# lgemc/WildlifeMapper

Measured on AMD Instinct MI355X. Metric: 1024x1024 tiles/sec (whole node), higher is better.
Workload: dtype fp16; 1 GPU; vit_h full path fft+encoder+decoder+PostProcess/NMS, fp16 MFMA, batch=16 tiles/GPU of 1024x1024x3 (BASELINE.json configs[2]); parallelism=dp1 tile shard, weights=seed 0 synthetic (random init), tolerance=logits within 1e-3 relative of the fp32 CPU forward, identical NMS index lists

## Files before the change

include/wm_hip.h:

```cpp
#ifndef WM_HIP_H
#define WM_HIP_H

#include <stdint.h>

#ifdef __cplusplus
extern "C" {
#endif

#define WM_ABI_VERSION 13

#define WM_PREC_BF16 0
#define WM_PREC_FP16 1
#define WM_PREC_FP8 2

#define WM_MAX_GLOBAL 8
#define WM_NUM_QUERIES 51
#define WM_NUM_LOGITS 8

typedef struct wm_config {
    int32_t embed_dim;
    int32_t depth;
    int32_t num_heads;
    int32_t num_global;
    int32_t global_attn_indexes[WM_MAX_GLOBAL];
// ... 32 lines not shown
int wm_abi_version(void);

int wm_create(const wm_config* cfg, int device, wm_handle** out);
int wm_destroy(wm_handle* h);
int wm_load_weight(wm_handle* h, const char* name, const float* host_data,
                   const int64_t* shape, int ndim);
int wm_finalize_weights(wm_handle* h);


int wm_preprocess_u8(const uint8_t* img_dev, float* out_dev, int batch, int height, int width, void* stream);

int wm_preprocess_u8_resized(const uint8_t* img_dev, float* out_dev, int batch, int height, int width, int size, int max_size,
                             void* stream);
int wm_resized_size(int height, int width, int size, int max_size, int* out_h, int* out_w);
int wm_debug_resize_coeffs(int in_size, int out_size, int* bounds_out, int* kk_out, int kk_capacity, int* ksize_out);

int wm_hfc_fft(wm_handle* h, const float* x_dev, float* hfc_dev, int batch, void* stream);

int wm_encoder_forward(wm_handle* h, const float* x_dev, const float* hfc_dev,
                       float* out_dev, int batch, void* stream);

int wm_decoder_forward(wm_handle* h, const float* emb_dev, float* logits_dev,
                       float* boxes_dev, int batch, void* stream);

int wm_postprocess_nms(wm_handle* h, const float* logits_dev, const float* boxes_dev,
                       const float* target_sizes_dev, float conf_thr, float score_thr,
                       float iou_thr, wm_box_record* records_dev, int batch, void* stream);

int wm_forward(wm_handle* h, const float* x_dev, const float* target_sizes_dev,
               float* logits_dev, float* boxes_dev, wm_box_record* records_dev,
               int batch, void* stream);

#define WM_CRITERION_MAX_TARGETS 2048
#define WM_CRITERION_SUMS 8
#define WM_CRITERION_NONFINITE 1
#define WM_CRITERION_UNSOLVED 2
int64_t wm_criterion_scratch_bytes(int batch, int total_targets);
int wm_criterion(wm_handle* h, const float* logits_dev, const float* boxes_dev, const float* tgt_boxes_dev,
                 const int32_t* tgt_labels_dev, const int32_t* tgt_offsets, int batch, float w_class, float w_bbox, float w_giou,
                 float eos_coef, void* scratch_dev, int64_t scratch_bytes, int32_t* match_dev, double* sums_dev,
                 int32_t* status_dev, float* cost_dev, double* dual_u_dev, double* dual_v_dev, void* stream);

typedef struct wm_frame_desc {
    const uint8_t* data;
    int32_t height, width;
} wm_frame_desc;
// ... 182 lines not shown
```

wildlifemapper_amd/_native.py:

```python
from __future__ import annotations

import ctypes as C
import os
from typing import Optional

import torch

_HERE = os.path.dirname(os.path.abspath(__file__))
LIB_PATH = os.environ.get("WM_HIP_LIB") or os.path.join(_HERE, "libwm_hip.so")

PREC_BF16, PREC_FP16, PREC_FP8 = 0, 1, 2
PREC_BY_NAME = {"bf16": PREC_BF16, "fp16": PREC_FP16, "f16": PREC_FP16, "fp8": PREC_FP8}
NUM_QUERIES, NUM_LOGITS = 51, 8
KCLASS_NAMES = ("gemm16", "attn_window", "attn_global", "layernorm", "other")
GEMM_VARIANTS = ("v1_128", "v2_160", "v2_128", "v3_lockstep", "v3_conv3x3", "v5_320", "v5_320_res", "v5_256", "v5_256_res",
                 "v5_320_lnf", "v5_256_lnf", "fp8_320", "fp8_256", "v5_320_foldp", "v5_256_foldp", "v5_320_split", "v5_256_split", "v3_patch_embed", "fp8_256_planes")
FLAG_CONF, FLAG_SCORE, FLAG_NMS, FLAG_MERGED = 1, 2, 4, 8
CRITERION_MAX_TARGETS, CRITERION_SUMS, CRITERION_NONFINITE, CRITERION_UNSOLVED = 2048, 8, 1, 2
CENSUS_MAX_DETS, CENSUS_SAME_CLASS, CENSUS_UNSOLVED = 262144, 1, 1
COVERAGE_MAX_SIDE, COVERAGE_MAX_CELLS, COVERAGE_MAX_FRAMES, COVERAGE_CLASSES, COVERAGE_STATS = 16384, 1 << 26, 65535, 7, 16
CFG_FUSE_LN = 1
CFG_FOLD_LN = 2
CFG_FOLD_LN_BF16 = 4
ABI_VERSION = 13
# ... 29 lines not shown
    "wm_finalize_weights": (_I, [_P]),
    "wm_preprocess_u8": (_I, [_P, _P, _I, _I, _I, _P]),
    "wm_preprocess_u8_resized": (_I, [_P, _P, _I, _I, _I, _I, _I, _P]),
    "wm_resized_size": (_I, [_I, _I, _I, _I, C.POINTER(_I), C.POINTER(_I)]),
    "wm_debug_resize_coeffs": (_I, [_I, _I, C.POINTER(_I), C.POINTER(_I), _I, C.POINTER(_I)]),
    "wm_tile_frames_u8": (_I, [_P, _I, _P, _P, _I, _P]),
    "wm_merge_frames_scratch_bytes": (_L, [_I]),
    "wm_merge_frames_nms": (_I, [_P, _P, C.POINTER(C.c_int32), _I, _F, _P, _L, _P, _P, _P, _P, _P]),
    "wm_merge_frames_fuse": (_I, [_P, _P, C.POINTER(C.c_int32), _I, _F, _P, _L, _P, _P, _P, _P, _P, _P, _P]),
    "wm_census_scratch_bytes": (_L, [_I]),
    "wm_census": (_I, [_P, _P, _P, _P, _I, _P, _I, C.c_double, _I, _P, _L, _P, _P, _P, _P, _P, _P]),
    "wm_coverage_raster": (_I, [_P, _P, _I, C.c_double, C.c_double, C.c_double, _I, _I, _P, _P, _P]),
    "wm_coverage_points": (_I, [_P, _P, _I, _P, _P, _I, C.c_double, C.c_double, C.c_double, _I, _I, _P, _P, _P, _P, _P]),
    "wm_resample_u8": (_I, [_P, _I, _I, _P, _I, _I, _P]),
    "wm_scaled_size": (_I, [_I, _I, C.c_double, C.POINTER(_I), C.POINTER(_I)]),
    "wm_chip_window": (_I, [C.POINTER(_F), _F, _I, _I, C.POINTER(C.c_int32)]),
    "wm_crop_chips_u8": (_I, [_P, _I, _P, _P, _I, _I, _F, _I, _I, _P, _P, _P]),
    "wm_box_outline_rect": (_I, [C.POINTER(_F), C.POINTER(C.c_int32)]),
    "wm_draw_boxes_u8": (_I, [_P, _I, _P, _P, _P, _I, _P, _I, _I, _P]),
    "wm_plot_image_u8": (_I, [_P, _I, _I, _I, _P, _P, _L, _P]),
    "wm_hfc_fft": (_I, [_P, _P, _P, _I, _P]),
    "wm_encoder_forward": (_I, [_P, _P, _P, _P, _I, _P]),
    "wm_decoder_forward": (_I, [_P, _P, _P, _P, _I, _P]),
    "wm_postprocess_nms": (_I, [_P, _P, _P, _P, _F, _F, _F, _P, _I, _P]),
    "wm_criterion_scratch_bytes": (_L, [_I, _I]),
    "wm_criterion": (_I, [_P, _P, _P, _P, _P, C.POINTER(C.c_int32), _I, _F, _F, _F, _F, _P, _L, _P, _P, _P, _P, _P, _P, _P]),
    "wm_forward": (_I, [_P, _P, _P, _P, _P, _P, _I, _P]),
    "wm_set_tap": (_I, [_P, _I]),
    "wm_read_tap": (_I, [_P, _P, _I, _P]),
    "wm_profile_enable": (_I, [_P, _I]),
    "wm_profile_reset": (_I, [_P]),
    "wm_profile_read": (_I, [_P, C.POINTER(WmKclassStat)]),
    "wm_debug_gemm_variant_counts": (_I, [C.POINTER(_L), _I]),
    "wm_debug_reset_gemm_variant_counts": (_I, []),
    "wm_debug_saturation_enable": (_I, [_P, _I]),
    "wm_debug_saturation_read": (_I, [_P, C.POINTER(_L), _I, _I, _P]),
    "wm_op_cvt_f32_to_16": (_I, [_P, _P, _L, _I, _P]),
    "wm_op_cvt_16_to_f32": (_I, [_P, _P, _L, _I, _P]),
    "wm_op_gemm16": (_I, [_P, _P, _P, _P, _I, _P, _P, _I, _I, _I, _I, _I, _P]),
    "wm_op_gemm16_takes_packed": (_I, [_I, _I, _I]),
    "wm_op_pack16": (_I, [_P, _P, _L, _I, _P]),
    "wm_op_ln_stats16": (_I, [_P, _P, _P, _L, _I, _I, _P]),
    "wm_op_ln_stats16_split": (_I, [_P, _P, _P, _P, _P, _L, _I, _I, _P]),
    "wm_op_gemm16_split": (_I, [_P, _P, _P, _P, _P, _P, _I, _I, _I, _I, _I, _P]),
    "wm_op_stream_merge": (_I, [_P, _P, _P, _L, _I, _I, _P]),
    "wm_op_unpack16": (_I, [_P, _P, _L, _I, _P]),
# ... 71 lines not shown
```

wildlifemapper_amd/csrc/gemm32.h:

```cpp
#pragma once
#include "wm_common.h"
#include "gemm_common.h"

namespace wm {

struct Gemm32Args {
    const float* A; const float* W; const float* bias; const float* residual; float* out;
    int M, N, K, act;
    int lda;
};

__global__ __launch_bounds__(256) void gemm32_kernel(Gemm32Args p) {
    constexpr int BM = 64, BN = 64, BK = 32, LD = BK + 1;
    __shared__ float sA[BM * LD];
    __shared__ float sW[BN * LD];
    const int tid = threadIdx.x, lane = tid & 63, wave = tid >> 6;
    const int wr = wave >> 1, wc = wave & 1;
    const int ntn = (p.N + BN - 1) / BN;
    const int lid = xcd_remap(blockIdx.x, gridDim.x);
    const int m0 = (lid / ntn) * BM, n0 = (lid % ntn) * BN;
    const int lrow = tid >> 2, lcol = (tid & 3) * 8;

    f32x16 acc;
#pragma unroll
// ... 30 lines not shown
    if (n >= p.N) return;
    const float bv = p.bias ? p.bias[n] : 0.f;
#pragma unroll
    for (int r = 0; r < 16; ++r) {
        const int m = m0 + wr * 32 + (r & 3) + 8 * (r >> 2) + 4 * (lane >> 5);
        if (m < p.M) {
            float v = acc[r] + bv;
            if (p.act == ACT_RELU) v = fmaxf(v, 0.f);
            else if (p.act == ACT_GELU) v = gelu_erf(v);
            else if (p.act == ACT_SIGMOID) v = 1.0f / (1.0f + expf(-v));
            if (p.residual) v += p.residual[(size_t)m * p.N + n];
            p.out[(size_t)m * p.N + n] = v;
        }
    }
}

constexpr float G32X3_WSCALE = 64.0f;
constexpr float G32X3_LOSCALE = 2048.0f;
struct Gemm32x3Args {
    const float* A; const float* W; const u16* Whi; const u16* Wlo;
    const float* bias; const float* residual; float* out;
    int M, N, K, act, lda;
    int* overflow;
};

__global__ __launch_bounds__(256) void split_w32_kernel(const float* __restrict__ w, u16* __restrict__ hi, u16* __restrict__ lo, int64_t n4, int* overflow) {
    for (int64_t i = (int64_t)blockIdx.x * 256 + threadIdx.x; i < n4; i += (int64_t)gridDim.x * 256) {
        const f32x4 v = *(const f32x4*)(w + i * 4) * G32X3_WSCALE;
        typename FP16::vec4 h, l;
        float amax = 0.f;
#pragma unroll
        for (int j = 0; j < 4; ++j) {
            h[j] = FP16::from_f32_bounded(v[j]);
            l[j] = FP16::from_f32_bounded((v[j] - FP16::to_f32(h[j])) * G32X3_LOSCALE);
            amax = fmaxf(amax, fabsf(v[j]));
        }
        *(typename FP16::vec4*)(hi + i * 4) = h;
        *(typename FP16::vec4*)(lo + i * 4) = l;
        if (amax >= 65504.f && overflow) *(volatile int*)overflow = 1;
    }
}

template <bool WPRE>
__global__ __launch_bounds__(256) void gemm32x3_kernel(Gemm32x3Args p) {
    constexpr int BM = 64, BN = 64, BK = 32, LDH = BK + 8;
    __shared__ __attribute__((aligned(16))) u16 sAh[BM * LDH], sAl[BM * LDH], sWh[BN * LDH], sWl[BN * LDH];
// ... 45 lines not shown
        else split8(s.w0, s.w1, G32X3_WSCALE, wh, wl);
        __syncthreads();
        *(uint4*)(sAh + lrow * LDH + lcol) = ah; *(uint4*)(sAl + lrow * LDH + lcol) = al;
        *(uint4*)(sWh + lrow * LDH + lcol) = wh; *(uint4*)(sWl + lrow * LDH + lcol) = wl;
        __syncthreads();
        if (kt + 2 < nk) fetch(s, (kt + 2) * BK);
#pragma unroll
        for (int ks = 0; ks < 2; ++ks) {
            const typename FP16::vec8 a_hi = *(const typename FP16::vec8*)(sAh + fa + 16 * ks), a_lo = *(const typename FP16::vec8*)(sAl + fa + 16 * ks);
            const typename FP16::vec8 w_hi = *(const typename FP16::vec8*)(sWh + fw + 16 * ks), w_lo = *(const typename FP16::vec8*)(sWl + fw + 16 * ks);
            accx = FP16::mfma32(a_lo, w_hi, accx);
            accx = FP16::mfma32(a_hi, w_lo, accx);
            acc = FP16::mfma32(a_hi, w_hi, acc);
        }
    };
    for (int kt = 0; kt < nk; kt += 2) {
        step(st[0], kt);
        if (kt + 1 < nk) step(st[1], kt + 1);
    }
    if (amax >= 65504.f && p.overflow) *(volatile int*)p.overflow = 1;

    const int n = n0 + wc * 32 + (lane & 31);
    if (n >= p.N) return;
    const float bv = p.bias ? p.bias[n] : 0.f;
#pragma unroll
    for (int r = 0; r < 16; ++r) {
        const int m = m0 + wr * 32 + (r & 3) + 8 * (r >> 2) + 4 * (lane >> 5);
        if (m < p.M) {
            float v = (acc[r] + accx[r] * (1.0f / G32X3_LOSCALE)) * (1.0f / G32X3_WSCALE) + bv;
            if (p.act == ACT_RELU) v = fmaxf(v, 0.f);
            else if (p.act == ACT_GELU) v = gelu_erf(v);
            else if (p.act == ACT_SIGMOID) v = 1.0f / (1.0f + expf(-v));
            if (p.residual) v += p.residual[(size_t)m * p.N + n];
            p.out[(size_t)m * p.N + n] = v;
        }
    }
}

}
```

wildlifemapper_amd/csrc/host_core.h:

```cpp
#pragma once
#include <hip/hip_runtime.h>

#include <cmath>
#include <cstdarg>
#include <cstdio>
#include <cstdlib>
#include <cstring>
#include <atomic>
#include <map>
#include <tuple>
#include <type_traits>
#include <mutex>
#include <set>
#include <string>
#include <algorithm>
#include <array>
#include <vector>

#include "../../include/wm_hip.h"
#include "wm_common.h"

#ifndef WM_DEV_TIMELINE
#define WM_DEV_TIMELINE 0
#endif
// ... 168 lines not shown
    std::map<const float*, std::pair<uint16_t*, uint16_t*>> w32x3;
    std::map<std::pair<const float*, int>, uint16_t*> bias16;
    float* mha_part = nullptr;
    size_t mha_part_cap = 0;
    bool row_major = false;
    bool sat_on = false;
    unsigned long long* sat_counts = nullptr;
    int tap_which = -2;
    float* tap_buf = nullptr;

    float *resid = nullptr, *tokbase = nullptr;
    uint16_t *xn16 = nullptr, *ao16 = nullptr, *qkv16 = nullptr, *hid16 = nullptr;
    uint16_t *p16 = nullptr, *h16 = nullptr, *he16 = nullptr, *hp16 = nullptr, *pt16 = nullptr, *q16 = nullptr,
             *kv16 = nullptr, *aoh16 = nullptr, *y1n16 = nullptr, *h1_16 = nullptr, *y2_16 = nullptr, *y2t16 = nullptr;
    float *pt32 = nullptr, *y1 = nullptr, *y1n32 = nullptr, *z32 = nullptr;
    float *n1 = nullptr, *n2 = nullptr, *emb_nhwc = nullptr, *emb_nchw = nullptr;
    uint16_t *n1n16 = nullptr, *x16last = nullptr;
    float *dkeys = nullptr, *dk_a = nullptr, *dk_b = nullptr, *dk_c = nullptr;
    float *dq = nullptr, *dt_q = nullptr, *dt_k = nullptr, *dt_v = nullptr, *dt_att = nullptr, *dt_hid = nullptr,
          *dt_h1 = nullptr, *dt_h2 = nullptr;
    float *logits = nullptr, *boxes = nullptr, *hfc = nullptr, *tsz_default = nullptr;
    float2 *fftR = nullptr, *fft_tw = nullptr;
    float* kpe = nullptr;
    wm_box_record* records = nullptr;
};

namespace {

template <class P>
int dalloc(wm_handle* h, P** out, size_t bytes) {
    void* p = nullptr;
    hipError_t e = hipMalloc(&p, bytes);
    if (e != hipSuccess) return fail("hipMalloc(%zu) failed: %s", bytes, hipGetErrorString(e));
    h->allocs.push_back(p);
    *out = (P*)p;
    return 0;
}

void dfree(wm_handle* h, void* p) {
    hipFree(p);
    for (auto& a : h->allocs) if (a == p) a = nullptr;
}

struct Bracket {
    wm_handle* h;
    hipStream_t s;
// ... 59 lines not shown
```

wildlifemapper_amd/csrc/host_decoder.h:

```cpp
#pragma once
#include "dec_kernels.h"
#include "host_encoder.h"

namespace {

struct DecAttnW { const float *wq, *bq, *wk, *bk, *wv, *bv, *wo, *bo; int internal; };

DecAttnW dec_w(wm_handle* h, const std::string& p, int internal) {
    return DecAttnW{W32(h, p + "q_proj.weight"), W32(h, p + "q_proj.bias"), W32(h, p + "k_proj.weight"), W32(h, p + "k_proj.bias"),
                    W32(h, p + "v_proj.weight"), W32(h, p + "v_proj.bias"), W32(h, p + "out_proj.weight"), W32(h, p + "out_proj.bias"), internal};
}

int decoder_impl(wm_handle* h, const float* keys_nhwc, float* logits, float* boxes, int B, hipStream_t s) {
    const std::string t = "mask_decoder.transformer.";
    const int E = OUTC, Mk = B * T, Mq = B * NQ;
    const float* tok = W32(h, "mask_decoder.mask_tokens.weight");
    float* keys = h->dkeys;
    HIP_TRY(hipMemcpyAsync(keys, keys_nhwc, (size_t)Mk * E * 4, hipMemcpyDeviceToDevice, s));
    float* queries = h->dq;
    WM_TRY(launch_simple(h, s, 0.0, add_bcast_kernel, dim3(grid_for((int64_t)Mq * E / 4)), dim3(256), (const float*)nullptr, tok, queries, (int64_t)Mq, E, NQ));

    auto add_q = [&](float* out) {
        return launch_simple(h, s, 0.0, add_bcast_kernel, dim3(grid_for((int64_t)Mq * E / 4)), dim3(256), (const float*)queries, tok, out, (int64_t)Mq, E, NQ);
    };
    auto add_k = [&](float* out) {
        return launch_simple(h, s, 0.0, add_bcast_kernel, dim3(grid_for((int64_t)Mk * E / 4)), dim3(256), (const float*)keys, (const float*)h->kpe, out, (int64_t)Mk, E, T);
    };
    auto ln = [&](float* x, const std::string& n, int rows) {
        return launch_layernorm(h, s, WM_PREC_FP16, x, W32(h, n + ".weight"), W32(h, n + ".bias"), 1e-5f, x, nullptr, rows, E);
    };
    auto token_to_image = [&](const DecAttnW& w, const float* kin) -> int {
        WM_TRY(add_q(h->dt_h1));
        WM_TRY(launch_gemm32(h, s, h->dt_h1, w.wq, w.bq, nullptr, h->dt_q, Mq, w.internal, E, ACT_NONE));
        WM_TRY(launch_gemm32(h, s, kin, w.wk, w.bk, nullptr, h->dk_a, Mk, w.internal, E, ACT_NONE));
        WM_TRY(launch_gemm32(h, s, keys, w.wv, w.bv, nullptr, h->dk_b, Mk, w.internal, E, ACT_NONE));
        WM_TRY(launch_mha32(h, s, h->dt_q, h->dk_a, h->dk_b, h->dt_att, B, 8, w.internal / 8, NQ, T));
// ... 26 lines not shown
            WM_TRY(add_q(h->dt_h1));
            WM_TRY(launch_gemm32(h, s, kpe_sum, w.wq, w.bq, nullptr, h->dk_a, Mk, w.internal, E, ACT_NONE));
            WM_TRY(launch_gemm32(h, s, h->dt_h1, w.wk, w.bk, nullptr, h->dt_k, Mq, w.internal, E, ACT_NONE));
            WM_TRY(launch_gemm32(h, s, queries, w.wv, w.bv, nullptr, h->dt_v, Mq, w.internal, E, ACT_NONE));
            WM_TRY(launch_mha32(h, s, h->dk_a, h->dt_k, h->dt_v, h->dk_c, B, 8, w.internal / 8, T, NQ));
            WM_TRY(launch_gemm32(h, s, h->dk_c, w.wo, w.bo, keys, keys, Mk, E, w.internal, ACT_NONE));
            WM_TRY(ln(keys, L + "norm4", Mk));
        }
    }
    WM_TRY(add_k(kpe_sum));
    WM_TRY(token_to_image(dec_w(h, t + "final_attn_token_to_image.", E / 2), kpe_sum));
    WM_TRY(ln(queries, t + "norm_final_attn", Mq));

    const std::string c = "mask_decoder.class_embed.layers.", bb = "mask_decoder.bbox_embed.layers.";
    WM_TRY(launch_gemm32(h, s, queries, W32(h, c + "0.weight"), W32(h, c + "0.bias"), nullptr, h->dt_h1, Mq, E, E, ACT_RELU));
    WM_TRY(launch_gemm32(h, s, h->dt_h1, W32(h, c + "1.weight"), W32(h, c + "1.bias"), nullptr, h->dt_h2, Mq, E, E, ACT_RELU));
    WM_TRY(launch_gemm32(h, s, h->dt_h2, W32(h, c + "2.weight"), W32(h, c + "2.bias"), nullptr, logits, Mq, WM_NUM_LOGITS, E, ACT_NONE));
    WM_TRY(launch_gemm32(h, s, queries, W32(h, bb + "0.weight"), W32(h, bb + "0.bias"), nullptr, h->dt_h1, Mq, E, E, ACT_RELU));
    WM_TRY(launch_gemm32(h, s, h->dt_h1, W32(h, bb + "1.weight"), W32(h, bb + "1.bias"), nullptr, h->dt_h2, Mq, E, E, ACT_RELU));
    WM_TRY(launch_gemm32(h, s, h->dt_h2, W32(h, bb + "2.weight"), W32(h, bb + "2.bias"), nullptr, boxes, Mq, 4, E, ACT_SIGMOID));
    return 0;
}

int forward_impl(wm_handle* h, const float* x_dev, const float* target_sizes_dev, float* logits_dev, float* boxes_dev,
                 wm_box_record* records_dev, int batch, hipStream_t s) {
    WM_TRY(fft_impl(h, x_dev, h->hfc, batch, s, true));
    WM_TRY(encoder_impl(h, x_dev, h->hfc, nullptr, batch, s, true));
    WM_TRY(decoder_impl(h, h->emb_nhwc, h->logits, h->boxes, batch, s));
    const float* ts = target_sizes_dev ? target_sizes_dev : h->tsz_default;
    WM_TRY(launch_simple(h, s, 0.0, postprocess_nms_kernel, dim3(batch), dim3(64), (const float*)h->logits, (const float*)h->boxes, ts,
                         0.05f, 0.5f, 0.4f, h->records));
    if (logits_dev) HIP_TRY(hipMemcpyAsync(logits_dev, h->logits, (size_t)batch * NQ * WM_NUM_LOGITS * 4, hipMemcpyDeviceToDevice, s));
    if (boxes_dev) HIP_TRY(hipMemcpyAsync(boxes_dev, h->boxes, (size_t)batch * NQ * 16, hipMemcpyDeviceToDevice, s));
    if (records_dev) HIP_TRY(hipMemcpyAsync(records_dev, h->records, (size_t)batch * NQ * sizeof(wm_box_record), hipMemcpyDeviceToDevice, s));
    return 0;
}

}
```

wildlifemapper_amd/csrc/host_gemm.h:

```cpp
#pragma once
#include "gemm16.h"
#include "gemm16_v2.h"
#include "gemm16_v3.h"
#include "gemm16_v5.h"
#include "gemm32.h"
#include "gemm8.h"
#include "misc_kernels.h"
#include "host_core.h"

namespace {

double gemm16_flops(const Gemm16Args& a) { return 2.0 * a.M * (double)a.N * a.K; }
double gemm16_bytes(const Gemm16Args& a) {
    return 2.0 * ((double)a.M * a.K + (double)a.N * a.K) + (a.out32 ? 4.0 : 0.0) * a.M * a.N + (a.out16 ? 2.0 : 0.0) * a.M * a.N +
           (a.residual ? 4.0 * (double)(a.res_mod > 0 ? a.res_mod : a.M) * a.N : 0.0);
}

template <class Kern, class Args>
int launch_gemm_kernel(wm_handle* h, hipStream_t s, Kern kern, int grid, int threads, int lds, const Args& a, int variant, double flops, double bytes) {
    WM_TRY(set_max_lds((const void*)kern, lds));
    if (variant >= 0) count_variant(variant);
    Bracket br(h, s, WM_KCLASS_GEMM16, flops, bytes);
    hipLaunchKernelGGL(kern, dim3(grid), dim3(threads), lds, s, a);
    HIP_TRY(hipGetLastError());
// ... 160 lines not shown
    });
}

int launch_patch_embed16(wm_handle* h, hipStream_t s, int prec, const void* img16, const void* W, const float* bias, const float* res, int res_mod,
                         float* out32, void* out16, int B, int N, int Cin) {
    const int M = B * 4096, K = Cin * 256;
    if (B <= 0 || (N % 320 && N % 256) || Cin <= 0) return fail("patch_embed: B=%d N=%d Cin=%d unsupported (N %% 320 or N %% 256)", B, N, Cin);
    if (!out32 && !out16) return fail("patch_embed: no output");
    Gemm16Args a{};
    a.A = (const u16*)img16; a.W = (const u16*)W; a.bias = bias; a.residual = res; a.out32 = out32; a.out16 = (u16*)out16;
    a.M = M; a.N = N; a.K = K; a.res_mod = res_mod; a.act = ACT_NONE; a.conv_c = Cin;
    count_variant(WM_GEMM_V3_PATCH);
    const double bytes = 2.0 * ((double)M * K + (double)N * K) + (out32 ? 4.0 : 0.0) * M * N + (out16 ? 2.0 : 0.0) * M * N;
    return by_type16(prec, [&](auto t) {
        return by_tile_width(N, [&](auto bn) {
            constexpr int BN = decltype(bn)::value;
            using G = G3<BN>;
            return launch_gemm_kernel(h, s, gemm16v3_kernel<decltype(t), BN, ALoad::PatchEmbed>, (M / 256) * (N / BN), G::THREADS, G::LDS, a, -1,
                                      2.0 * M * (double)N * K, bytes);
        });
    });
}

int launch_gemm32(wm_handle* h, hipStream_t s, const float* A, const float* W, const float* bias, const float* res,
                  float* out, int M, int N, int K, int act, int lda = 0, int mode = 0) {
    if (K % 16) return fail("gemm32: K=%d must be a multiple of 16", K);
    static const bool f32_only = getenv("WM_GEMM32_F32") && atoi(getenv("WM_GEMM32_F32")) != 0;
    if ((mode == 2 || mode == 3) && K % 32) return fail("gemm32 (split form): K=%d must be a multiple of 32", K);
    if (mode == 2 || mode == 3 || (mode == 0 && h && !f32_only && K % 32 == 0)) {
        Gemm32x3Args a{A, W, nullptr, nullptr, bias, res, out, M, N, K, act, lda > 0 ? lda : K, h ? h->overflow + 1 : nullptr};
        if (mode == 3) {
            const size_t n = (size_t)N * K;
            void* pb = nullptr;
            WM_TRY(op_scratch(s, 3, n * 4, &pb));
            u16* hi = (u16*)pb;
            hipLaunchKernelGGL(split_w32_kernel, dim3(grid_for((int64_t)n / 4)), dim3(256), 0, s, W, hi, hi + n, (int64_t)n / 4, (int*)nullptr);
            HIP_TRY(hipGetLastError());
            a.Whi = hi; a.Wlo = hi + n;
        }
        if (mode == 0) {
            auto it = h->w32x3.find(W);
            if (it == h->w32x3.end()) {
                uint16_t *hi = nullptr, *lo = nullptr;
                const size_t n = (size_t)N * K;
                if (n % 4) return fail("gemm32: weight of %zu elements", n);
                WM_TRY(dalloc(h, &hi, n * 2)); WM_TRY(dalloc(h, &lo, n * 2));
                hipLaunchKernelGGL(split_w32_kernel, dim3(grid_for((int64_t)n / 4)), dim3(256), 0, s, W, (u16*)hi, (u16*)lo, (int64_t)n / 4, h->overflow + 1);
                HIP_TRY(hipGetLastError());
                it = h->w32x3.emplace(W, std::make_pair(hi, lo)).first;
            }
            a.Whi = (const u16*)it->second.first; a.Wlo = (const u16*)it->second.second;
        }
        Bracket br(h, s, WM_KCLASS_OTHER, 2.0 * M * (double)N * K, 4.0 * ((double)M * K + (double)M * N) + 4.0 * (double)N * K);
// ... 15 lines not shown
```

wildlifemapper_amd/csrc/host_weights.h:

```cpp
#pragma once
#include "misc_kernels.h"
#include "fft_kernels.h"
#include "host_core.h"

namespace {

bool ends_with(const std::string& s, const char* suf) {
    const size_t n = strlen(suf);
    return s.size() >= n && s.compare(s.size() - n, n, suf) == 0;
}

static inline uint16_t f32_to_bf16_host(float f) {
    uint32_t u;
    memcpy(&u, &f, 4);
    if ((u & 0x7fffffffu) > 0x7f800000u) return (uint16_t)((u >> 16) | 0x40);
    u += 0x7fffu + ((u >> 16) & 1u);
    return (uint16_t)(u >> 16);
}

static inline uint16_t f32_to_f16_host(float f) {
    _Float16 h = (_Float16)fminf(fmaxf(f, -65504.f), 65504.f);
    uint16_t r;
    memcpy(&r, &h, 2);
    return r;
}

static inline uint8_t f32_to_e4m3_host(float f) {
    if (f != f) return 0x7f;
// ... 349 lines not shown
                HIP_TRY(hipMemcpy(d32, w.data.data(), n * 4, hipMemcpyHostToDevice));
                h->wsrc32[name] = d32;
            }
        } else {
            WM_TRY(upload32(h, name, w.data.data(), n));
        }
    }
    if (h->staged.count("prompt_encoder.pe_layer.positional_encoding_gaussian_matrix")) {
        const HostW& g = h->staged["prompt_encoder.pe_layer.positional_encoding_gaussian_matrix"];
        const int F = OUTC / 2;
        std::vector<float> pe((size_t)T * OUTC);
        for (int y = 0; y < GRID; ++y)
            for (int x = 0; x < GRID; ++x) {
                const float cx = 2.0f * ((x + 0.5f) / GRID) - 1.0f, cy = 2.0f * ((y + 0.5f) / GRID) - 1.0f;
                for (int f = 0; f < F; ++f) {
                    float arg = cx * g.data[f] + cy * g.data[F + f];
                    arg = arg * 6.283185307179586f;
                    pe[(size_t)(y * GRID + x) * OUTC + f] = (float)sin((double)arg);
                    pe[(size_t)(y * GRID + x) * OUTC + F + f] = (float)cos((double)arg);
                }
            }
        HIP_TRY(hipMemcpy(h->kpe, pe.data(), pe.size() * 4, hipMemcpyHostToDevice));
    }
    if (h->fold && h->enc_ready) {
        for (int i = 0; i < h->depth; ++i) {
            const std::string b = "image_encoder.blocks." + std::to_string(i) + ".";
            const int P = block_prec(h, i) == WM_PREC_FP8 ? WM_PREC_BF16 : block_prec(h, i);
            const std::pair<const char*, const char*> pairs[] = {{"attn.qkv", "norm1"}, {"mlp.lin1", "norm2"}};
            for (const auto& pr : pairs) {
                const std::string wn = b + pr.first + ".weight";
                if (!h->w16.count(wn)) continue;
                const int N = (int)h->expected.at(wn)[0], K = (int)h->expected.at(wn)[1];
                if (!h->wfold.count(wn)) {
                    uint16_t* wf = nullptr; float *c1 = nullptr, *c2 = nullptr;
                    WM_TRY(dalloc(h, &wf, (size_t)N * K * 2)); WM_TRY(dalloc(h, &c1, (size_t)N * 4)); WM_TRY(dalloc(h, &c2, (size_t)N * 4));
                    h->wfold[wn] = wf; h->fold_c1[wn] = c1; h->fold_c2[wn] = c2;
                }
                const float* g = h->w32.at(b + pr.second + ".weight");
                const float* be = h->w32.at(b + pr.second + ".bias");
                const float* bias = h->w32.at(b + pr.first + ".bias");
                WM_TRY(launch_fold_weight(0, P, h->w16.at(wn), h->fold_from16 ? nullptr : h->wsrc32.at(wn), g, be, bias, h->wfold[wn], h->fold_c1[wn], h->fold_c2[wn], N, K));
            }
        }
    }
    HIP_TRY(hipDeviceSynchronize());
    h->staged.clear();
// ... 6 lines not shown
```

wildlifemapper_amd/csrc/wm_api.hip:

```cpp
#include "host_core.h"
#if WM_DEV_TIMELINE
#include "host_dev_timeline.h"
#endif
#include "host_gemm.h"
#include "host_norm.h"
#include "host_attn.h"
#include "host_weights.h"
#include "host_encoder.h"
#include "host_decoder.h"
#include "host_frontend.h"
#include "host_criterion.h"

extern "C" const char* wm_last_error(void) { return g_err; }
extern "C" int wm_abi_version(void) { return WM_ABI_VERSION; }

extern "C" int wm_create(const wm_config* cfg, int device, wm_handle** out) {
    if (!cfg || !out) return fail("wm_create: null argument");
    if (cfg->embed_dim <= 0 || cfg->num_heads <= 0 || cfg->embed_dim % cfg->num_heads) return fail("wm_create: bad dims");
    if (cfg->depth <= 0 || cfg->depth > 64) return fail("wm_create: depth %d out of range", cfg->depth);
    if (cfg->max_batch <= 0) return fail("wm_create: max_batch must be positive");
    if (cfg->embed_dim % 256 || cfg->embed_dim > 1280) return fail("wm_create: embed_dim %d unsupported (multiple of 256, <= 1280)", cfg->embed_dim);
    const int hd = cfg->embed_dim / cfg->num_heads;
    if (hd != 64 && hd != 80) return fail("wm_create: head_dim %d unsupported (64 or 80)", hd);
    if (cfg->precision != WM_PREC_BF16 && cfg->precision != WM_PREC_FP16 && cfg->precision != WM_PREC_FP8) return fail("wm_create: bad precision");
// ... 75 lines not shown

extern "C" int wm_hfc_fft(wm_handle* h, const float* x_dev, float* hfc_dev, int batch, void* stream) {
    if (!h) return fail("wm_hfc_fft: null handle");
    if (batch <= 0 || batch > h->maxB) return fail("wm_hfc_fft: batch %d outside 1..%d", batch, h->maxB);
    if (!x_dev || !hfc_dev) return fail("wm_hfc_fft: null buffer");
    HIP_TRY(hipSetDevice(h->device));
    return fft_impl(h, x_dev, hfc_dev, batch, (hipStream_t)stream);
}

extern "C" int wm_encoder_forward(wm_handle* h, const float* x_dev, const float* hfc_dev, float* out_dev, int batch, void* stream) {
    WM_TRY(check_ready(h, batch, "wm_encoder_forward", true, false));
    if (!x_dev || !hfc_dev || !out_dev) return fail("wm_encoder_forward: null buffer");
    return encoder_impl(h, x_dev, hfc_dev, out_dev, batch, (hipStream_t)stream);
}

extern "C" int wm_decoder_forward(wm_handle* h, const float* emb_dev, float* logits_dev, float* boxes_dev, int batch, void* stream) {
    WM_TRY(check_ready(h, batch, "wm_decoder_forward", false, true));
    if (!emb_dev || !logits_dev || !boxes_dev) return fail("wm_decoder_forward: null buffer");
    hipStream_t s = (hipStream_t)stream;
    WM_TRY(launch_simple(h, s, batch * 8.4e6, transpose32_kernel, dim3(T / 64, OUTC / 64, batch), dim3(256), emb_dev, h->emb_nhwc, OUTC, T));
    return decoder_impl(h, h->emb_nhwc, logits_dev, boxes_dev, batch, s);
}

extern "C" int wm_postprocess_nms(wm_handle* h, const float* logits_dev, const float* boxes_dev, const float* target_sizes_dev,
                                  float conf_thr, float score_thr, float iou_thr, wm_box_record* records_dev, int batch, void* stream) {
    if (batch <= 0) return fail("wm_postprocess_nms: batch %d", batch);
    if (!logits_dev || !boxes_dev || !target_sizes_dev || !records_dev) return fail("wm_postprocess_nms: null buffer");
    if (h) HIP_TRY(hipSetDevice(h->device));
    return launch_simple(h, (hipStream_t)stream, 0.0, postprocess_nms_kernel, dim3(batch), dim3(64), logits_dev, boxes_dev,
                         target_sizes_dev, conf_thr, score_thr, iou_thr, records_dev);
}

extern "C" int wm_forward(wm_handle* h, const float* x_dev, const float* target_sizes_dev, float* logits_dev, float* boxes_dev,
                          wm_box_record* records_dev, int batch, void* stream) {
    WM_TRY(check_ready(h, batch, "wm_forward", true, true));
    if (!x_dev) return fail("wm_forward: null input");
    return forward_impl(h, x_dev, target_sizes_dev, logits_dev, boxes_dev, records_dev, batch, (hipStream_t)stream);
}

extern "C" int64_t wm_criterion_scratch_bytes(int batch, int total_targets) { return criterion_scratch_bytes(batch, total_targets); }

extern "C" int wm_criterion(wm_handle* h, const float* logits_dev, const float* boxes_dev, const float* tgt_boxes_dev,
                            const int32_t* tgt_labels_dev, const int32_t* tgt_offsets, int batch, float w_class, float w_bbox, float w_giou,
                            float eos_coef, void* scratch_dev, int64_t scratch_bytes, int32_t* match_dev, double* sums_dev,
                            int32_t* status_dev, float* cost_dev, double* dual_u_dev, double* dual_v_dev, void* stream) {
    if (h) HIP_TRY(hipSetDevice(h->device));
// ... 355 lines not shown
```

Baseline: 171.3 tiles/s.

## Precompute decoder positional-encoding projections and fuse K/V projections in mask decoder

Precomputes the weight-only parts of the mask decoder at weight-finalize time: positional-encoding and token projections become per-row addend tables, and the first self-attention over the constant mask tokens runs once into a tokens0 constant. The gemm32 epilogue gains a per-row addend table and a split second output, so each token-to-image K and V projection over the image keys runs as one GEMM instead of separate add and projection passes. This removes redundant per-batch work on the constant path and some launches. In exchange it adds stored tables, a more complex epilogue that preloads residuals, and a rounding order that differs slightly from the reference.

After: 172.0 tiles/s (median of 6 runs). Within noise of the previous version (+0.4%).

```diff
diff --git a/include/wm_hip.h b/include/wm_hip.h
--- a/include/wm_hip.h
+++ b/include/wm_hip.h
@@ -78,6 +78,9 @@
 
 int wm_decoder_forward(wm_handle* h, const float* emb_dev, float* logits_dev,
                        float* boxes_dev, int batch, void* stream);
+
+int wm_debug_decoder_kv(wm_handle* h, int which, const float* keys_dev, float* k_out_dev, float* v_out_dev, int fused,
+                        int batch, void* stream);
 
 int wm_postprocess_nms(wm_handle* h, const float* logits_dev, const float* boxes_dev,
                        const float* target_sizes_dev, float conf_thr, float score_thr,
diff --git a/wildlifemapper_amd/_native.py b/wildlifemapper_amd/_native.py
--- a/wildlifemapper_amd/_native.py
+++ b/wildlifemapper_amd/_native.py
@@ -75,6 +75,7 @@
     "wm_hfc_fft": (_I, [_P, _P, _P, _I, _P]),
     "wm_encoder_forward": (_I, [_P, _P, _P, _P, _I, _P]),
     "wm_decoder_forward": (_I, [_P, _P, _P, _P, _I, _P]),
+    "wm_debug_decoder_kv": (_I, [_P, _I, _P, _P, _P, _I, _I, _P]),
     "wm_postprocess_nms": (_I, [_P, _P, _P, _P, _F, _F, _F, _P, _I, _P]),
     "wm_criterion_scratch_bytes": (_L, [_I, _I]),
     "wm_criterion": (_I, [_P, _P, _P, _P, _P, C.POINTER(C.c_int32), _I, _F, _F, _F, _F, _P, _L, _P, _P, _P, _P, _P, _P, _P]),
diff --git a/wildlifemapper_amd/csrc/gemm32.h b/wildlifemapper_amd/csrc/gemm32.h
--- a/wildlifemapper_amd/csrc/gemm32.h
+++ b/wildlifemapper_amd/csrc/gemm32.h
@@ -76,6 +76,8 @@
     const float* bias; const float* residual; float* out;
     int M, N, K, act, lda;
     int* overflow;
+    const float* rowadd; int rowadd_mod, rowadd_n;
+    float* out2; int nsplit;
 };
 
 __global__ __launch_bounds__(256) void split_w32_kernel(const float* __restrict__ w, u16* __restrict__ hi, u16* __restrict__ lo, int64_t n4, int* overflow) {
@@ -167,19 +169,46 @@
 
     const int n = n0 + wc * 32 + (lane & 31);
     if (n >= p.N) return;
-    const float bv = p.bias ? p.bias[n] : 0.f;
+    const int wave_u = __builtin_amdgcn_readfirstlane(wave);
+    const bool tab = p.rowadd && n0 + (wave_u & 1) * 32 < p.rowadd_n;
+    float add[16];
+    if (tab) {
+        const int mb = (m0 + (wave_u >> 1) * 32) % p.rowadd_mod;
+#pragma unroll
+        for (int r = 0; r < 16; ++r) {
+            int row = mb + (r & 3) + 8 * (r >> 2) + 4 * (lane >> 5);
+            if (row >= p.rowadd_mod) row -= p.rowadd_mod;
+            add[r] = p.rowadd[(size_t)row * p.rowadd_n + n];
+        }
+    } else {
+        const float bv = p.bias ? p.bias[n] : 0.f;
+#pragma unroll
+        for (int r = 0; r < 16; ++r) add[r] = bv;
+    }
+    float rs[16];
+#pragma unroll
+    for (int r = 0; r < 16; ++r) {
+        const int m = min(m0 + wr * 32 + (r & 3) + 8 * (r >> 2) + 4 * (lane >> 5), p.M - 1);
+        rs[r] = p.residual ? p.residual[(size_t)m * p.N + n] : 0.f;
+    }
+    float* op = p.out;
+    int ldo = p.N, no = n;
+    if (p.out2) {
+        if (n >= p.nsplit) { op = p.out2; ldo = p.N - p.nsplit; no = n - p.nsplit; }
+        else ldo = p.nsplit;
+    }
 #pragma unroll
     for (int r = 0; r < 16; ++r) {
         const int m = m0 + wr * 32 + (r & 3) + 8 * (r >> 2) + 4 * (lane >> 5);
         if (m < p.M) {
-            float v = (acc[r] + accx[r] * (1.0f / G32X3_LOSCALE)) * (1.0f / G32X3_WSCALE) + bv;
+            float v = (acc[r] + accx[r] * (1.0f / G32X3_LOSCALE)) * (1.0f / G32X3_WSCALE) + add[r];
             if (p.act == ACT_RELU) v = fmaxf(v, 0.f);
             else if (p.act == ACT_GELU) v = gelu_erf(v);
             else if (p.act == ACT_SIGMOID) v = 1.0f / (1.0f + expf(-v));
-            if (p.residual) v += p.residual[(size_t)m * p.N + n];
-            p.out[(size_t)m * p.N + n] = v;
-        }
-    }
-}
-
-}
+            if (p.residual) v += rs[r];
+            op[(size_t)m * ldo + no] = v;
+        }
+    }
+}
+
+}
diff --git a/wildlifemapper_amd/csrc/host_core.h b/wildlifemapper_amd/csrc/host_core.h
--- a/wildlifemapper_amd/csrc/host_core.h
+++ b/wildlifemapper_amd/csrc/host_core.h
@@ -214,6 +214,8 @@
     float *logits = nullptr, *boxes = nullptr, *hfc = nullptr, *tsz_default = nullptr;
     float2 *fftR = nullptr, *fft_tw = nullptr;
     float* kpe = nullptr;
+    std::map<std::string, float*> dconst;
+    std::set<std::string> dconst_bad;
     wm_box_record* records = nullptr;
 };
 
diff --git a/wildlifemapper_amd/csrc/host_dec_tables.h b/wildlifemapper_amd/csrc/host_dec_tables.h
--- /dev/null
+++ b/wildlifemapper_amd/csrc/host_dec_tables.h
@@ -0,0 +1,62 @@
+#pragma once
+#include <string>
+#include <vector>
+
+namespace wm_dec {
+
+enum Kind { KEY_TABLE, TOKEN_TABLE, CONCAT_W, CONCAT_B, TOKENS0 };
+
+struct Derived {
+    Kind kind;
+    std::string key;
+    std::vector<std::string> src;
+    int n;
+};
+
+inline const char* gaussian_name() { return "prompt_encoder.pe_layer.positional_encoding_gaussian_matrix"; }
+inline const char* tokens_name() { return "mask_decoder.mask_tokens.weight"; }
+inline const char* tokens0_key() { return "mask_decoder.tokens0"; }
+inline std::string table_key(const std::string& proj) { return proj + ".pe_const"; }
+inline std::string concat_key(const std::string& attn, const char* what) { return attn + "kv_proj." + what; }
+
+inline std::vector<std::string> token_to_image_attns() {
+    const std::string t = "mask_decoder.transformer.";
+    return {t + "layers.0.cross_attn_token_to_image.", t + "layers.1.cross_attn_token_to_image.", t + "final_attn_token_to_image."};
+}
+
+inline std::vector<Derived> plan(int embed = 256) {
+    const std::string t = "mask_decoder.transformer.";
+    std::vector<Derived> p;
+    auto table = [&](Kind k, const std::string& proj, int n) {
+        p.push_back(Derived{k, table_key(proj), {proj + ".weight", proj + ".bias", k == KEY_TABLE ? gaussian_name() : tokens_name()}, n});
+    };
+    for (const std::string& a : token_to_image_attns()) {
+        table(KEY_TABLE, a + "k_proj", embed / 2);
+        table(TOKEN_TABLE, a + "q_proj", embed / 2);
+        p.push_back(Derived{CONCAT_W, concat_key(a, "weight"), {a + "k_proj.weight", a + "v_proj.weight"}, embed});
+        p.push_back(Derived{CONCAT_B, concat_key(a, "bias"), {a + "k_proj.bias", a + "v_proj.bias"}, embed});
+    }
+    for (int i = 0; i < 2; ++i) {
+        const std::string a = t + "layers." + std::to_string(i) + ".cross_attn_image_to_token.";
+        table(KEY_TABLE, a + "q_proj", embed / 2);
+        table(TOKEN_TABLE, a + "k_proj", embed / 2);
+    }
+    table(TOKEN_TABLE, t + "layers.1.self_attn.q_proj", embed);
+    table(TOKEN_TABLE, t + "layers.1.self_attn.k_proj", embed);
+    Derived t0{TOKENS0, tokens0_key(), {tokens_name()}, embed};
+    for (const char* n : {"q_proj", "k_proj", "v_proj", "out_proj"})
+        for (const char* w : {".weight", ".bias"}) t0.src.push_back(t + "layers.0.self_attn." + n + w);
+    for (const char* w : {".weight", ".bias"}) t0.src.push_back(t + "layers.0.norm1" + w);
+    p.push_back(t0);
+    return p;
+}
+
+template <class Staged, class Built>
+bool stale(const Derived& d, const Staged& staged, const Built& built) {
+    if (!built.count(d.key)) return true;
+    for (const std::string& s : d.src)
+        if (staged.count(s)) return true;
+    return false;
+}
+
+}
diff --git a/wildlifemapper_amd/csrc/host_decoder.h b/wildlifemapper_amd/csrc/host_decoder.h
--- a/wildlifemapper_amd/csrc/host_decoder.h
+++ b/wildlifemapper_amd/csrc/host_decoder.h
@@ -11,7 +11,7 @@
                     W32(h, p + "v_proj.weight"), W32(h, p + "v_proj.bias"), W32(h, p + "out_proj.weight"), W32(h, p + "out_proj.bias"), internal};
 }
 
-int decoder_impl(wm_handle* h, const float* keys_nhwc, float* logits, float* boxes, int B, hipStream_t s) {
+int decoder_unfused_impl(wm_handle* h, const float* keys_nhwc, float* logits, float* boxes, int B, hipStream_t s) {
     const std::string t = "mask_decoder.transformer.";
     const int E = OUTC, Mk = B * T, Mq = B * NQ;
     const float* tok = W32(h, "mask_decoder.mask_tokens.weight");
@@ -84,6 +84,146 @@
     return 0;
 }
 
+const float* DCONST(wm_handle* h, const std::string& n) { return h->dconst.at(n); }
+
+int dec_self_attn0(wm_handle* h, hipStream_t s, float* queries, int B) {
+    const std::string L = "mask_decoder.transformer.layers.0.";
+    const int E = OUTC, Mq = B * NQ;
+    const DecAttnW w = dec_w(h, L + "self_attn.", E);
+    WM_TRY(launch_gemm32(h, s, queries, w.wq, w.bq, nullptr, h->dt_q, Mq, E, E, ACT_NONE));
+    WM_TRY(launch_gemm32(h, s, queries, w.wk, w.bk, nullptr, h->dt_k, Mq, E, E, ACT_NONE));
+    WM_TRY(launch_gemm32(h, s, queries, w.wv, w.bv, nullptr, h->dt_v, Mq, E, E, ACT_NONE));
+    WM_TRY(launch_mha32(h, s, h->dt_q, h->dt_k, h->dt_v, h->dt_att, B, 8, E / 8, NQ, NQ));
+    WM_TRY(launch_gemm32(h, s, h->dt_att, w.wo, w.bo, nullptr, queries, Mq, E, E, ACT_NONE));
+    return launch_layernorm(h, s, WM_PREC_FP16, queries, W32(h, L + "norm1.weight"), W32(h, L + "norm1.bias"), 1e-5f, queries, nullptr, Mq, E);
+}
+
+int dec_build_derived(wm_handle* h) {
+    if (gemm32_f32_only()) return 0;
+    const hipStream_t s = 0;
+    const int E = OUTC;
+    for (const wm_dec::Derived& d : wm_dec::plan(E)) {
+        if (!wm_dec::stale(d, h->staged, h->dconst)) continue;
+        const int rows = d.kind == wm_dec::KEY_TABLE ? T : d.kind == wm_dec::CONCAT_W ? d.n : d.kind == wm_dec::CONCAT_B ? 1 : NQ;
+        const int cols = d.kind == wm_dec::CONCAT_W ? E : d.n;
+        if (!h->dconst.count(d.key)) {
+            float* p = nullptr;
+            WM_TRY(dalloc(h, &p, (size_t)rows * cols * 4));
+            h->dconst[d.key] = p;
+        }
+        float* out = h->dconst.at(d.key);
+        HIP_TRY(hipDeviceSynchronize());
+        volatile int* ovf = (volatile int*)h->overflow + 1;
+        const int ovf_before = *ovf;
+        *ovf = 0;
+        switch (d.kind) {
+            case wm_dec::KEY_TABLE:
+            case wm_dec::TOKEN_TABLE:
+                WM_TRY(launch_gemm32(h, s, d.kind == wm_dec::KEY_TABLE ? h->kpe : W32(h, wm_dec::tokens_name()), W32(h, d.src[0]), W32(h, d.src[1]),
+                                     nullptr, out, rows, d.n, E, ACT_NONE));
+                break;
+            case wm_dec::CONCAT_W:
+            case wm_dec::CONCAT_B: {
+                const size_t half = (size_t)rows * cols / 2 * 4;
+                HIP_TRY(hipMemcpyAsync(out, W32(h, d.src[0]), half, hipMemcpyDeviceToDevice, s));
+                HIP_TRY(hipMemcpyAsync((char*)out + half, W32(h, d.src[1]), half, hipMemcpyDeviceToDevice, s));
+                break;
+            }
+            case wm_dec::TOKENS0:
+                HIP_TRY(hipMemcpyAsync(out, W32(h, wm_dec::tokens_name()), (size_t)NQ * E * 4, hipMemcpyDeviceToDevice, s));
+                WM_TRY(dec_self_attn0(h, s, out, 1));
+                break;
+        }
+        HIP_TRY(hipDeviceSynchronize());
+        if (*ovf) h->dconst_bad.insert(d.key);
+        else h->dconst_bad.erase(d.key);
+        *ovf = ovf_before;
+    }
+    return 0;
+}
+
+int dec_project_kv(wm_handle* h, hipStream_t s, const std::string& attn, const float* keys, float* k_out, float* v_out, int Mk, bool fused) {
+    const int E = OUTC, I = E / 2;
+    Gemm32Ext x;
+    x.rowadd = DCONST(h, wm_dec::table_key(attn + "k_proj")); x.rowadd_mod = T; x.rowadd_n = I;
+    if (!fused) {
+        WM_TRY(launch_gemm32(h, s, keys, W32(h, attn + "k_proj.weight"), nullptr, nullptr, k_out, Mk, I, E, ACT_NONE, 0, 0, &x));
+        return launch_gemm32(h, s, keys, W32(h, attn + "v_proj.weight"), W32(h, attn + "v_proj.bias"), nullptr, v_out, Mk, I, E, ACT_NONE);
+    }
+    x.out2 = v_out; x.nsplit = I;
+    return launch_gemm32(h, s, keys, DCONST(h, wm_dec::concat_key(attn, "weight")), DCONST(h, wm_dec::concat_key(attn, "bias")), nullptr, k_out,
+                         Mk, E, E, ACT_NONE, 0, 0, &x);
+}
+
+int decoder_impl(wm_handle* h, const float* keys_nhwc, float* logits, float* boxes, int B, hipStream_t s) {
+    if (gemm32_f32_only()) return decoder_unfused_impl(h, keys_nhwc, logits, boxes, B, s);
+    const std::string t = "mask_decoder.transformer.";
+    const int E = OUTC, Mk = B * T, Mq = B * NQ;
+    const float* keys = keys_nhwc;
+    float* queries = h->dq;
+    if (!h->dconst_bad.empty()) ((volatile int*)h->overflow)[1] = 1;
+    WM_TRY(launch_simple(h, s, 0.0, add_bcast_kernel, dim3(grid_for((int64_t)Mq * E / 4)), dim3(256), (const float*)nullptr,
+                         DCONST(h, wm_dec::tokens0_key()), queries, (int64_t)Mq, E, NQ));
+
+    auto ln = [&](float* x, const std::string& n, int rows) {
+        return launch_layernorm(h, s, WM_PREC_FP16, x, W32(h, n + ".weight"), W32(h, n + ".bias"), 1e-5f, x, nullptr, rows, E);
+    };
+    auto proj_pe = [&](const float* a, const std::string& proj, int per, float* out, int M, int N) {
+        Gemm32Ext x;
+        x.rowadd = DCONST(h, wm_dec::table_key(proj)); x.rowadd_mod = per; x.rowadd_n = N;
+        return launch_gemm32(h, s, a, W32(h, proj + ".weight"), nullptr, nullptr, out, M, N, E, ACT_NONE, 0, 0, &x);
+    };
+    auto token_to_image = [&](const std::string& a) -> int {
+        const DecAttnW w = dec_w(h, a, E / 2);
+        WM_TRY(proj_pe(queries, a + "q_proj", NQ, h->dt_q, Mq, w.internal));
+        WM_TRY(dec_project_kv(h, s, a, keys, h->dk_a, h->dk_b, Mk, true));
+        WM_TRY(launch_mha32(h, s, h->dt_q, h->dk_a, h->dk_b, h->dt_att, B, 8, w.internal / 8, NQ, T));
+        WM_TRY(launch_gemm32(h, s, h->dt_att, w.wo, w.bo, queries, queries, Mq, E, w.internal, ACT_NONE));
+        return 0;
+    };
+
+    for (int i = 0; i < 2; ++i) {
+        const std::string L = t + "layers." + std::to_string(i) + ".";
+        if (i != 0) {
+            const std::string a = L + "self_attn.";
+            const DecAttnW w = dec_w(h, a, E);
+            WM_TRY(proj_pe(queries, a + "q_proj", NQ, h->dt_q, Mq, E));
+            WM_TRY(proj_pe(queries, a + "k_proj", NQ, h->dt_k, Mq, E));
+            WM_TRY(launch_gemm32(h, s, queries, w.wv, w.bv, nullptr, h->dt_v, Mq, E, E, ACT_NONE));
+            WM_TRY(launch_mha32(h, s, h->dt_q, h->dt_k, h->dt_v, h->dt_att, B, 8, E / 8, NQ, NQ));
+            WM_TRY(launch_gemm32(h, s, h->dt_att, w.wo, w.bo, queries, queries, Mq, E, E, ACT_NONE));
+            WM_TRY(ln(queries, L + "norm1", Mq));
+        }
+        WM_TRY(token_to_image(L + "cross_attn_token_to_image."));
+        WM_TRY(ln(queries, L + "norm2", Mq));
+        WM_TRY(launch_gemm32(h, s, queries, W32(h, L + "mlp.lin1.weight"), W32(h, L + "mlp.lin1.bias"), nullptr, h->dt_hid, Mq, DEC_MLP, E, ACT_RELU));
+        WM_TRY(launch_gemm32(h, s, h->dt_hid, W32(h, L + "mlp.lin2.weight"), W32(h, L + "mlp.lin2.bias"), queries, queries, Mq, E, DEC_MLP, ACT_NONE));
+        WM_TRY(ln(queries, L + "norm3", Mq));
+        {
+            const std::string a = L + "cross_attn_image_to_token.";
+            const DecAttnW w = dec_w(h, a, E / 2);
+            WM_TRY(proj_pe(keys, a + "q_proj", T, h->dk_a, Mk, w.internal));
+            WM_TRY(proj_pe(queries, a + "k_proj", NQ, h->dt_k, Mq, w.internal));
+            WM_TRY(launch_gemm32(h, s, queries, w.wv, w.bv, nullptr, h->dt_v, Mq, w.internal, E, ACT_NONE));
+            WM_TRY(launch_mha32(h, s, h->dk_a, h->dt_k, h->dt_v, h->dk_c, B, 8, w.internal / 8, T, NQ));
+            WM_TRY(launch_gemm32(h, s, h->dk_c, w.wo, w.bo, keys, h->dkeys, Mk, E, w.internal, ACT_NONE));
+            WM_TRY(ln(h->dkeys, L + "norm4", Mk));
+            keys = h->dkeys;
+        }
+    }
+    WM_TRY(token_to_image(t + "final_attn_token_to_image."));
+    WM_TRY(ln(queries, t + "norm_final_attn", Mq));
+
+    const std::string c = "mask_decoder.class_embed.layers.", bb = "mask_decoder.bbox_embed.layers.";
+    WM_TRY(launch_gemm32(h, s, queries, W32(h, c + "0.weight"), W32(h, c + "0.bias"), nullptr, h->dt_h1, Mq, E, E, ACT_RELU));
+    WM_TRY(launch_gemm32(h, s, h->dt_h1, W32(h, c + "1.weight"), W32(h, c + "1.bias"), nullptr, h->dt_h2, Mq, E, E, ACT_RELU));
+    WM_TRY(launch_gemm32(h, s, h->dt_h2, W32(h, c + "2.weight"), W32(h, c + "2.bias"), nullptr, logits, Mq, WM_NUM_LOGITS, E, ACT_NONE));
+    WM_TRY(launch_gemm32(h, s, queries, W32(h, bb + "0.weight"), W32(h, bb + "0.bias"), nullptr, h->dt_h1, Mq, E, E, ACT_RELU));
+    WM_TRY(launch_gemm32(h, s, h->dt_h1, W32(h, bb + "1.weight"), W32(h, bb + "1.bias"), nullptr, h->dt_h2, Mq, E, E, ACT_RELU));
+    WM_TRY(launch_gemm32(h, s, h->dt_h2, W32(h, bb + "2.weight"), W32(h, bb + "2.bias"), nullptr, boxes, Mq, 4, E, ACT_SIGMOID));
+    return 0;
+}
+
 int forward_impl(wm_handle* h, const float* x_dev, const float* target_sizes_dev, float* logits_dev, float* boxes_dev,
                  wm_box_record* records_dev, int batch, hipStream_t s) {
     WM_TRY(fft_impl(h, x_dev, h->hfc, batch, s, true));
diff --git a/wildlifemapper_amd/csrc/host_gemm.h b/wildlifemapper_amd/csrc/host_gemm.h
--- a/wildlifemapper_amd/csrc/host_gemm.h
+++ b/wildlifemapper_amd/csrc/host_gemm.h
@@ -206,13 +206,29 @@
     });
 }
 
+bool gemm32_f32_only() {
+    static const bool f32_only = getenv("WM_GEMM32_F32") && atoi(getenv("WM_GEMM32_F32")) != 0;
+    return f32_only;
+}
+
+struct Gemm32Ext {
+    const float* rowadd = nullptr; int rowadd_mod = 0, rowadd_n = 0;
+    float* out2 = nullptr; int nsplit = 0;
+};
+
 int launch_gemm32(wm_handle* h, hipStream_t s, const float* A, const float* W, const float* bias, const float* res,
-                  float* out, int M, int N, int K, int act, int lda = 0, int mode = 0) {
+                  float* out, int M, int N, int K, int act, int lda = 0, int mode = 0, const Gemm32Ext* ext = nullptr) {
     if (K % 16) return fail("gemm32: K=%d must be a multiple of 16", K);
-    static const bool f32_only = getenv("WM_GEMM32_F32") && atoi(getenv("WM_GEMM32_F32")) != 0;
+    const bool f32_only = gemm32_f32_only();
+    if (ext) {
+        if (mode != 0 || !h || f32_only || K % 32) return fail("gemm32: the per-token addend and the second output exist only in the engine's split form");
+        if (ext->rowadd && (ext->rowadd_mod < 32 || ext->rowadd_n <= 0 || ext->rowadd_n > N || ext->rowadd_n % 32)) return fail("gemm32: addend of %d rows, %d columns", ext->rowadd_mod, ext->rowadd_n);
+        if (ext->out2 && (res || ext->nsplit <= 0 || ext->nsplit >= N || ext->nsplit % 64)) return fail("gemm32: second output from column %d of %d", ext->nsplit, N);
+    }
     if ((mode == 2 || mode == 3) && K % 32) return fail("gemm32 (split form): K=%d must be a multiple of 32", K);
     if (mode == 2 || mode == 3 || (mode == 0 && h && !f32_only && K % 32 == 0)) {
-        Gemm32x3Args a{A, W, nullptr, nullptr, bias, res, out, M, N, K, act, lda > 0 ? lda : K, h ? h->overflow + 1 : nullptr};
+        Gemm32x3Args a{A, W, nullptr, nullptr, bias, res, out, M, N, K, act, lda > 0 ? lda : K, h ? h->overflow + 1 : nullptr, nullptr, 1, 0, nullptr, 0};
+        if (ext) { a.rowadd = ext->rowadd; a.rowadd_mod = ext->rowadd ? ext->rowadd_mod : 1; a.rowadd_n = ext->rowadd_n; a.out2 = ext->out2; a.nsplit = ext->nsplit; }
         if (mode == 3) {
             const size_t n = (size_t)N * K;
             void* pb = nullptr;
diff --git a/wildlifemapper_amd/csrc/host_weights.h b/wildlifemapper_amd/csrc/host_weights.h
--- a/wildlifemapper_amd/csrc/host_weights.h
+++ b/wildlifemapper_amd/csrc/host_weights.h
@@ -2,8 +2,11 @@
 #include "misc_kernels.h"
 #include "fft_kernels.h"
 #include "host_core.h"
+#include "host_dec_tables.h"
 
 namespace {
+
+int dec_build_derived(wm_handle* h);
 
 bool ends_with(const std::string& s, const char* suf) {
     const size_t n = strlen(suf);
@@ -399,6 +402,7 @@
             }
         HIP_TRY(hipMemcpy(h->kpe, pe.data(), pe.size() * 4, hipMemcpyHostToDevice));
     }
+    if (h->dec_ready) WM_TRY(dec_build_derived(h));
     if (h->fold && h->enc_ready) {
         for (int i = 0; i < h->depth; ++i) {
             const std::string b = "image_encoder.blocks." + std::to_string(i) + ".";
diff --git a/wildlifemapper_amd/csrc/wm_api.hip b/wildlifemapper_amd/csrc/wm_api.hip
--- a/wildlifemapper_amd/csrc/wm_api.hip
+++ b/wildlifemapper_amd/csrc/wm_api.hip
@@ -121,6 +121,15 @@
     return decoder_impl(h, h->emb_nhwc, logits_dev, boxes_dev, batch, s);
 }
 
+extern "C" int wm_debug_decoder_kv(wm_handle* h, int which, const float* keys_dev, float* k_out_dev, float* v_out_dev, int fused,
+                                   int batch, void* stream) {
+    WM_TRY(check_ready(h, batch, "wm_debug_decoder_kv", false, true));
+    if (!keys_dev || !k_out_dev || !v_out_dev) return fail("wm_debug_decoder_kv: null buffer");
+    if (which < 0 || which > 2) return fail("wm_debug_decoder_kv: attention %d outside 0..2", which);
+    if (gemm32_f32_only()) return fail("wm_debug_decoder_kv: WM_GEMM32_F32=1 runs the decoder as a chain of single ops");
+    return dec_project_kv(h, (hipStream_t)stream, wm_dec::token_to_image_attns()[which], keys_dev, k_out_dev, v_out_dev, batch * T, fused != 0);
+}
+
 extern "C" int wm_postprocess_nms(wm_handle* h, const float* logits_dev, const float* boxes_dev, const float* target_sizes_dev,
                                   float conf_thr, float score_thr, float iou_thr, wm_box_record* records_dev, int batch, void* stream) {
     if (batch <= 0) return fail("wm_postprocess_nms: batch %d", batch);
```
